# tomisetsu/mochi-db

Hardware: AMD Instinct MI355X
Metric: verified grant signatures/sec (1/2/4/8 GPU) + % of INT32 VALU roofline (higher is better)
Workload: dtype u32

## Files before the change

mochi-db_amd/csrc/capi.cpp:

```cpp
#include <hip/hip_runtime.h>
#include <openssl/bn.h>
#include <openssl/core_names.h>
#include <openssl/evp.h>
#include <openssl/pem.h>

#include <cstdarg>
#include <cstdio>
#include <cstring>
#include <condition_variable>
#include <mutex>
#include <thread>
#include <string>
#include <vector>

#include "../../include/mochi_hip.h"
#include "kernels.h"
#include "mont.h"
#include "w2.h"
#include "w2_encode.h"
#include "w2_host.h"

namespace {

thread_local std::string g_err;
// ... 199 lines not shown
  BN_CTX_free(ctx);
  if (!ok) return fail(MOCHI_EINVAL, "fold matrix precompute failed");
  for (int mt = 0; mt < kFoldMT; mt++)
    for (int ks = 0; ks < kFoldKS; ks++)
      for (int lane = 0; lane < 64; lane++)
        for (int jj = 0; jj < 16; jj++) {
          const int row = 32 * mt + (lane & 31), limb = 8 * ks + 4 * (lane >> 5) + jj / 4;
          if (row < kRows && limb < kFoldNH)
            f->img[((mt * kFoldKS + ks) * 64 + lane) * 16 + jj] = W[(size_t)row * kK + 4 * limb + jj % 4];
        }
  return MOCHI_OK;
}

}

namespace mochi {
const uint32_t* ctx_last_accept_dev(mochi_ctx* c, uint32_t* words, int* device, hipStream_t* stream);
int set_error(int code, const std::string& msg) {
  g_err = msg;
  return code;
}
}

struct mochi_ctx {
  std::mutex ref_mu;
  int batcher_refs = 0;
  bool destroy_pending = false;
  int device = 0;
  hipStream_t stream = nullptr;
  uint32_t n_keys = 0;
  mochi::KeyEntry* d_keys = nullptr;
  mochi::FoldKey* d_fold = nullptr;
  std::mutex mu;
  DevBuf digest, ts, hash_off, hash_len, flags, count, cursor, total, perm, xbuf, dedup, lead;
  DevBuf dev_in, dev_out;
  PinnedBuf pin_in, pin_out;
  hipStream_t s_in = nullptr, s_out = nullptr;
  hipStream_t aux = nullptr;
  hipEvent_t ev_fork = nullptr, ev_join = nullptr;
  hipEvent_t ev_scratch = nullptr;
  bool scratch_used = false;
  hipStream_t scratch_st = nullptr;
  std::vector<hipEvent_t> chunk_ev;
  std::vector<hipEvent_t> tot_ev;
  hipEvent_t evs[2][4] = {{nullptr, nullptr, nullptr, nullptr}, {nullptr, nullptr, nullptr, nullptr}};
  hipEvent_t* ev = evs[0];
  int ev_set = 0, ev_done = 0;
  float last_ms[3] = {0, 0, 0};
  float last_total_ms = 0;
  bool timing_pending = false;
  uint32_t chunk_grants = 0;
  uint32_t small_grants = 4096;
  DevBuf ids, id_off;
  uint32_t n_ids = 0;
  std::vector<std::string> server_ids;
  DevBuf w2_cnt, w2_status, w2_scan, w2_goff, w2_glen, w2_sig, w2_signer, w2_gkey, w2_okey, w2_oflags, w2_sigsrc,
      w2_mgo, w2_ots, w2_okoff, w2_oklen, w2_same;
  PinnedBuf w2_tot;
  hipEvent_t ev_tot = nullptr;
  DevBuf w2e_scratch, w2e_scan;
  PinnedBuf w2e_tot;
  std::vector<hipEvent_t> w2e_ev;
  bool w2e_ev_valid = false;
  const uint32_t* acc_dev = nullptr;
  uint32_t acc_words = 0;
  uint64_t gen = 0;
  bool profiling = false;
// ... 254 lines not shown
  a.blob = b->grant_bytes;
  a.grant_off = b->grant_off;
  a.grant_len = b->grant_len;
  a.sig = b->sig;
  a.signer = b->signer;
  a.grant_key = b->grant_key;
  a.cert_grant_off = b->cert_grant_off;
  a.cert_op_off = b->cert_op_off;
  a.op_key = b->op_key;
  a.op_flags = b->op_flags;
  a.expected_hash = b->expected_hash;
  a.cert_mg_off = b->cert_mg_off;
  a.mg_grant_off = b->mg_grant_off;
  a.op_object_ts = b->op_object_ts;
  a.op_key_off = b->op_key_off;
  a.op_key_len = b->op_key_len;
  a.quorum_mode = p->quorum_mode;
  const uint32_t R = p->replication_factor;
  a.majority = 2 * (R / 3) + 1;
  a.strict_gt = p->strict_gt ? 1 : 0;
  a.keys = c->d_keys;
  a.fold = c->d_fold;
  a.digest = c->digest.as<uint32_t>();
  a.n_dist = N + C;
  a.lead = c->lead.as<uint32_t>();
  a.ts = o->grant_ts ? o->grant_ts : c->ts.as<int64_t>();
  a.hash_off = c->hash_off.as<uint64_t>();
  a.hash_len = c->hash_len.as<uint32_t>();
  a.flags = o->grant_flags ? o->grant_flags : c->flags.as<uint8_t>();
  a.count = c->count.as<uint32_t>();
  a.cursor = c->cursor.as<uint32_t>();
  a.total = c->total.as<uint32_t>();
  a.perm = c->perm.as<uint32_t>();
  a.xbuf = c->xbuf.as<uint32_t>();
  a.rare = c->dedup.as<uint8_t>();
  a.small_grants = c->small_grants;
  a.grant_same = grant_same;
  a.grant_valid_bits = o->grant_valid_bits;
  a.cert_accept_bits = o->cert_accept_bits;
  a.cert_reason = o->cert_reason;
  a.cert_fail_op = o->cert_fail_op;
  a.op_decision = o->op_decision;
  a.op_g0 = o->op_g0;
  a.op_ts = o->op_ts;
  a.op_out_off = op_out_off;
  a.msg_status = msg_status;
  a.aux = prep_serial() ? nullptr : c->aux;
  a.ev_fork = c->ev_fork;
  a.ev_join = c->ev_join;
  if (c->profiling) {
    std::vector<hipEvent_t> evs(2 * mochi::kProfStages, nullptr);
    for (auto& e : evs) HIP_TRY(hipEventCreate(&e));
    c->prof_sets.push_back(evs);
    a.prof_events = c->prof_sets.back().data();
  }
  HIP_TRY(scratch_acquire(c, st));
  HIP_TRY(mochi::launch_verify(a, st));
  HIP_TRY(scratch_release(c, st));
  return MOCHI_OK;
}

bool is_pinned(const void* ptr) {
  if (!ptr) return false;
  hipPointerAttribute_t a;
  if (hipPointerGetAttributes(&a, ptr) != hipSuccess) {
    (void)hipGetLastError();
// ... 2 lines not shown
  return a.type == hipMemoryTypeHost;
}

void par_memcpy(void* dst, const void* src, size_t n) {
  constexpr size_t kPar = 8u << 20;
  if (n < kPar) {
    memcpy(dst, src, n);
    return;
  }
  const unsigned hw = std::thread::hardware_concurrency();
  const unsigned nt = hw < 2 ? 1 : hw > 8 ? 8 : hw;
  const size_t per = (n + nt - 1) / nt;
  std::vector<std::thread> th;
  for (unsigned t = 1; t < nt; t++) {
    const size_t lo = t * per;
    if (lo >= n) break;
    const size_t len = per < n - lo ? per : n - lo;
    th.emplace_back([=] { memcpy((char*)dst + lo, (const char*)src + lo, len); });
  }
  memcpy(dst, src, per < n ? per : n);
  for (auto& x : th) x.join();
}

int ensure_scratch(mochi_ctx* c, uint32_t N, uint32_t C) {
  const uint64_t slots = mochi::slot_capacity(N, c->n_keys);
  const size_t ND = (size_t)N + C;
  int rc;
  if ((rc = c->digest.ensure(sizeof(uint32_t) * 8 * ND)) || (rc = c->dedup.ensure((size_t)N)) ||
      (rc = c->ts.ensure(sizeof(int64_t) * (size_t)N)) || (rc = c->hash_off.ensure(sizeof(uint64_t) * ND)) ||
      (rc = c->hash_len.ensure(sizeof(uint32_t) * ND)) || (rc = c->flags.ensure((size_t)N)) ||
      (rc = c->lead.ensure(sizeof(uint32_t) * (size_t)N)) ||
      (rc = c->count.ensure(sizeof(uint32_t) * c->n_keys)) || (rc = c->cursor.ensure(sizeof(uint32_t) * c->n_keys)) ||
      (rc = c->total.ensure(mochi::kTotalWords * sizeof(uint32_t))) || (rc = c->perm.ensure(sizeof(uint32_t) * (size_t)slots)) ||
      (rc = c->xbuf.ensure(sizeof(uint32_t) * mochi::kL * (size_t)slots)))
    return rc;
  return MOCHI_OK;
}

enum Seg {
  kBlob, kGrantOff, kGrantLen, kSig, kSigner, kGrantKey, kCertGrantOff, kCertOpOff, kOpKey, kOpFlags, kExpHash,
  kCertMgOff, kMgGrantOff, kOpObjTs, kOpKeyOff, kOpKeyLen, kNumSeg
};

int run_host_pipeline(mochi_ctx* c, const mochi_batch* b, const mochi_params* p, mochi_verdicts* o) {
  const uint32_t N = b->n_grants, C = b->n_certs, O = b->n_ops;
  c->acc_dev = nullptr;
  c->acc_words = 0;
  const bool mg = b->cert_mg_off != nullptr;
  struct Chunk {
    uint32_t c0, c1, g0, g1, o0, o1, m0, m1;
    uint64_t lo, hi;
    size_t seg[kNumSeg];
  };
  std::vector<Chunk> ch;
  uint32_t max_grants = 0, max_certs = 0;
  for (uint32_t c0 = 0; c0 < C || (C == 0 && ch.empty());) {
    uint32_t c1 = c0;
    do c1 = c1 + 32 < C ? c1 + 32 : C;
    while (c1 < C && b->cert_grant_off[c1] - b->cert_grant_off[c0] < c->chunk_grants);
    Chunk k{};
    k.c0 = c0;
    k.c1 = c1;
    k.g0 = b->cert_grant_off[c0];
    k.g1 = b->cert_grant_off[c1];
    k.o0 = b->cert_op_off[c0];
    k.o1 = b->cert_op_off[c1];
// ... 991 lines not shown
  c->acc_words = 0;
  return rc;
}

int mochi_fold_matrix(const uint8_t* modulus_be, int8_t* img, uint32_t* cadd) {
  if (!modulus_be || !img || !cadd) return fail(MOCHI_EINVAL, "null argument");
  if (!(modulus_be[0] & 0x80) || !(modulus_be[255] & 1)) return fail(MOCHI_EINVAL, "modulus must be odd, 2048 bits");
  std::vector<mochi::FoldKey> f(1);
  int rc = make_fold_key(modulus_be, f.data());
  if (rc) return rc;
  memcpy(img, f[0].img, sizeof f[0].img);
  memcpy(cadd, f[0].cadd, sizeof f[0].cadd);
  return MOCHI_OK;
}

int mochi_rsa_public_op(mochi_ctx* c, uint32_t n, const uint8_t* sig_be, const uint16_t* signer, uint8_t* out_be,
                        uint32_t* out_z) {
  if (!c || (n && (!sig_be || !signer || !out_be))) return fail(MOCHI_EINVAL, "null argument");
  for (uint32_t i = 0; i < n; i++)
    if (signer[i] >= c->n_keys) return fail(MOCHI_EINVAL, "signer[%u] out of range", i);
  if (n == 0) return MOCHI_OK;
  std::lock_guard<std::mutex> lk(c->mu);
  new_call(c);
  int save = 0;
  (void)hipGetDevice(&save);
  if (hipSetDevice(c->device) != hipSuccess) return fail(MOCHI_EHIP, "hipSetDevice(%d)", c->device);
  const uint64_t slots = mochi::slot_capacity(n, c->n_keys);
  const size_t sig_bytes = (size_t)MOCHI_RSA_BYTES * n, y_bytes = sizeof(uint32_t) * 64 * (size_t)n;
  int rc;
  if ((rc = c->dev_in.ensure(align_up(sig_bytes, 256) + sizeof(uint16_t) * n)) || (rc = c->dev_out.ensure(y_bytes)) ||
      (rc = c->digest.ensure(sizeof(uint32_t) * 8 * (size_t)n)) || (rc = c->flags.ensure(n)) ||
      (rc = c->count.ensure(sizeof(uint32_t) * c->n_keys)) || (rc = c->cursor.ensure(sizeof(uint32_t) * c->n_keys)) ||
      (rc = c->total.ensure(mochi::kTotalWords * sizeof(uint32_t))) || (rc = c->perm.ensure(sizeof(uint32_t) * (size_t)slots)) ||
      (rc = c->xbuf.ensure(sizeof(uint32_t) * mochi::kL * (size_t)slots))) {
    (void)hipSetDevice(save);
    return rc;
  }
  hipStream_t st = c->stream;
  uint8_t* din = c->dev_in.as<uint8_t>();
  uint16_t* dsigner = (uint16_t*)(din + align_up(sig_bytes, 256));
  mochi::LaunchArgs a;
  memset(&a, 0, sizeof a);
  a.n_grants = n;
  a.n_keys = c->n_keys;
  a.n_slots = (uint32_t)slots;
  a.sig = din;
  a.signer = dsigner;
  a.keys = c->d_keys;
  a.fold = c->d_fold;
  a.digest = c->digest.as<uint32_t>();
  a.flags = c->flags.as<uint8_t>();
  a.count = c->count.as<uint32_t>();
  a.cursor = c->cursor.as<uint32_t>();
  a.total = c->total.as<uint32_t>();
  a.perm = c->perm.as<uint32_t>();
  a.xbuf = c->xbuf.as<uint32_t>();
  a.dbg_y = c->dev_out.as<uint32_t>();
  a.skip_prep_tally = true;
  a.small_grants = c->small_grants;
  std::vector<uint32_t> y(64 * (size_t)n), perm, z;
  bool ok = hipMemcpyAsync(din, sig_be, sig_bytes, hipMemcpyHostToDevice, st) == hipSuccess &&
            hipMemcpyAsync(dsigner, signer, sizeof(uint16_t) * n, hipMemcpyHostToDevice, st) == hipSuccess &&
            hipMemsetAsync(a.digest, 0, sizeof(uint32_t) * 8 * (size_t)n, st) == hipSuccess &&
            hipMemsetAsync(a.flags, 0, n, st) == hipSuccess && mochi::launch_verify(a, st) == hipSuccess &&
            hipMemcpyAsync(y.data(), a.dbg_y, y_bytes, hipMemcpyDeviceToHost, st) == hipSuccess;
  if (ok && out_z) {
    perm.resize(slots);
    z.resize((size_t)mochi::kL * slots);
    ok = hipMemcpyAsync(perm.data(), a.perm, sizeof(uint32_t) * slots, hipMemcpyDeviceToHost, st) == hipSuccess &&
         hipMemcpyAsync(z.data(), a.xbuf, sizeof(uint32_t) * z.size(), hipMemcpyDeviceToHost, st) == hipSuccess;
  }
  ok = ok && hipStreamSynchronize(st) == hipSuccess;
  (void)hipSetDevice(save);
  if (!ok) return fail(MOCHI_EHIP, "rsa_public_op failed: %s", hipGetErrorString(hipGetLastError()));
  for (uint32_t g = 0; g < n; g++)
    for (int i = 0; i < 64; i++) {
      const uint32_t w = y[(size_t)g * 64 + i];
      uint8_t* o = out_be + (size_t)g * 256 + 256 - 4 * (i + 1);
      o[0] = (uint8_t)(w >> 24);
      o[1] = (uint8_t)(w >> 16);
      o[2] = (uint8_t)(w >> 8);
      o[3] = (uint8_t)w;
    }
  if (out_z)
    for (uint64_t sl = 0; sl < slots; sl++) {
      const uint32_t g = perm[sl];
      if (g == 0xFFFFFFFFu) continue;
      for (int j = 0; j < mochi::kL; j++) out_z[(size_t)g * mochi::kL + j] = z[(size_t)j * slots + sl];
// ... 404 lines not shown
```

mochi-db_amd/csrc/fold_dev.h:

```cpp
#pragma once
#include <atomic>

#include "fold.h"
#include "kara_dev.h"
#include "mont.h"

namespace mochi {

typedef int v4i __attribute__((ext_vector_type(4)));
typedef int v16i __attribute__((ext_vector_type(16)));

__device__ __forceinline__ void swap32(int& a, int& b) {
  const auto r = __builtin_amdgcn_permlane32_swap(a, b, false, false);
  a = r[0];
  b = r[1];
}

__device__ __forceinline__ int64_t mad_i64(int32_t a, int32_t b, int64_t c) {
  int64_t d;
  uint64_t cc;
  asm("v_mad_i64_i32 %0, %1, %2, %3, %4" : "=v"(d), "=s"(cc) : "v"(a), "s"(b), "v"(c));
  return d;
}

constexpr int kHL = 10;

typedef __attribute__((address_space(1))) char gchar;
typedef __attribute__((address_space(1))) uint32_t guint;

template <bool SUB_H, bool BIASED = false>
__device__ __forceinline__ void fold_reduce(const uint32_t (&t)[2 * kL], uint32_t (&x)[kL],
                                            const v4i* __restrict__ wl, cptr cadd, const uint32_t* hl) {
  v4i a = wl[0];
  v4i b0[kFoldKS], b1[kFoldKS];
// ... 187 lines not shown
        __syncthreads();
        const v4i* src = (const v4i*)fold[key].img;
        for (uint32_t i = threadIdx.x; i < kFoldImgBytes / 16; i += blockDim.x) w[i] = src[i];
        __syncthreads();
        cur_key = key;
      }
      fn(base, key, g_lead);
    }
    if (dyn) {
      it ^= 1;
      if (threadIdx.x == 0) s_grp[it] = nxt;
      __syncthreads();
      grp = __builtin_amdgcn_readfirstlane(s_grp[it]);
    } else {
      grp++;
    }
  }
}

inline uint32_t fold_grid(uint32_t n_slots) {
  static std::atomic<int> n_cu[64];
  int dev = 0;
  (void)hipGetDevice(&dev);
  uint32_t cus = 256u;
  if (dev >= 0 && dev < 64) {
    int v = n_cu[dev].load(std::memory_order_relaxed);
    if (v == 0) {
      if (hipDeviceGetAttribute(&v, hipDeviceAttributeMultiprocessorCount, dev) != hipSuccess || v <= 0) v = 256;
      n_cu[dev].store(v, std::memory_order_relaxed);
    }
    cus = (uint32_t)v;
  }
  const uint32_t groups = (n_slots + kBucketAlign - 1) / kBucketAlign;
  return groups < cus ? groups : cus;
}

}
```

mochi-db_amd/csrc/kernels.h:

```cpp
#pragma once
#include <hip/hip_runtime.h>
#include <stdint.h>

#include "fold.h"

namespace mochi {

struct KeyEntry;

struct LaunchArgs {
  uint32_t n_grants, n_certs, n_keys, n_slots;
  const uint8_t* blob;
  const uint64_t* grant_off;
  const uint32_t* grant_len;
  const uint8_t* sig;
  const uint16_t* signer;
  const uint8_t* grant_key;
  const uint32_t* cert_grant_off;
  const uint32_t* cert_op_off;
  const uint8_t* op_key;
  const uint8_t* op_flags;
  const uint8_t* expected_hash;
  const uint32_t* cert_mg_off;
  const uint32_t* mg_grant_off;
  const int64_t* op_object_ts;
  const uint64_t* op_key_off;
  const uint32_t* op_key_len;
  uint32_t majority, strict_gt, quorum_mode;
  const KeyEntry* keys;
  const FoldKey* fold;
  uint32_t* digest;
  int64_t* ts;
  uint64_t* hash_off;
  uint32_t* hash_len;
  uint32_t* lead;
  uint32_t n_dist;
  uint8_t* flags;
  uint32_t* count;
  uint32_t* cursor;
  uint32_t* total;
  uint8_t* rare;
  const uint32_t* grant_same;
  uint32_t* perm;
  uint32_t* xbuf;
  uint32_t* grant_valid_bits;
  uint32_t* cert_accept_bits;
  uint8_t* cert_reason;
  uint8_t* cert_fail_op;
  uint8_t* op_decision;
  uint32_t* op_g0;
  int64_t* op_ts;
  const uint32_t* op_out_off;
  const uint8_t* msg_status;
  uint32_t* dbg_y;
  bool skip_prep_tally;
  uint32_t small_grants;
  hipStream_t aux;
  hipEvent_t ev_fork, ev_join;
  hipEvent_t* prof_events;
};

enum TotalWord { kTotSlots = 0, kTotPowGroup, kTotFinalGroup, kTotalWords = 4 };

enum ProfStage { kStagePrep = 0, kStageBucket, kStagePow, kStageFinal, kStageTally, kProfStages };

inline uint64_t slot_capacity(uint32_t n_grants, uint32_t n_keys) {
  return (uint64_t)n_grants + (uint64_t)kBucketAlign * (n_keys < n_grants ? n_keys : n_grants);
}

hipError_t launch_verify(const LaunchArgs& a, hipStream_t stream);

size_t sign_key_bytes();
void sign_key_set(void* dst, const uint32_t* p, const uint32_t* q, const uint32_t* r3p, const uint32_t* r3q,
                  const uint32_t* qinv_r, const uint32_t* dp, const uint32_t* dq, const uint32_t* cpad, uint32_t p0inv,
                  uint32_t q0inv, uint32_t dp_bits, uint32_t dq_bits);
hipError_t launch_rsa_sign(const uint8_t* blob, const uint64_t* goff, const uint32_t* glen, uint32_t n,
                           const void* key, uint8_t* sig, uint32_t fault_idx, hipStream_t stream);
hipError_t launch_withhold(const uint8_t* flags, uint32_t n, uint8_t* sig, uint32_t* rejected, hipStream_t stream);
hipError_t launch_pack_bits(const uint8_t* flags, uint32_t n, uint8_t mask, uint32_t* bits, hipStream_t stream);
void launch_rsa_pow(const LaunchArgs& a, hipStream_t stream, bool latency = false);
void launch_rsa_final(const LaunchArgs& a, const uint32_t* lead, uint32_t n_dist, hipStream_t stream,
                      bool latency = false);
void launch_rsa_raw(const LaunchArgs& a, hipStream_t stream);

}
```

mochi-db_amd/csrc/kernels.hip:

```cpp
#include <hip/hip_runtime.h>
#include <stdint.h>
#include <stdlib.h>

#include "../../include/mochi_hip.h"
#include "kernels.h"
#include "prep_dev.h"
#include "proto_dev.h"

namespace mochi {


#ifndef MOCHI_PREP_WAVES
#define MOCHI_PREP_WAVES 4
#endif
#if MOCHI_PREP_WAVES
#define MOCHI_PREP_ATTR __attribute__((amdgpu_waves_per_eu(MOCHI_PREP_WAVES)))
#else
#define MOCHI_PREP_ATTR
#endif
__global__ __launch_bounds__(256) MOCHI_PREP_ATTR void k_grant_prep(const PrepArgs a) {
  const uint32_t i = blockIdx.x * blockDim.x + threadIdx.x;
  if (i < a.n) grant_prep_one(a, i);
}

struct PrepCertArgs {
  const uint8_t* grant_key;
  const uint32_t* cert_grant_off;
  const uint32_t* same;
  uint32_t n_certs;
  uint8_t* rare;
  const uint8_t* expected;
};

__device__ __forceinline__ uint32_t leader_hash_word(const PrepArgs& a, const PrepCertArgs& p, uint32_t c,
                                                     uint64_t og, const PrepOut& o) {
// ... 302 lines not shown
    run += (count[k] + kBucketAlign - 1) & ~(kBucketAlign - 1);
  }
}

#ifndef MOCHI_SCATTER_PER
#define MOCHI_SCATTER_PER 16
#endif
constexpr uint32_t kScatterPer = MOCHI_SCATTER_PER;

__global__ __launch_bounds__(256) void k_bucket_scatter(const uint16_t* __restrict__ signer, uint32_t n, uint32_t n_keys,
                                                        uint32_t* __restrict__ cursor, uint32_t* __restrict__ perm) {
  extern __shared__ uint32_t lds[];
  uint32_t* lcount = lds;
  uint32_t* lbase = lds + n_keys;
  for (uint32_t k = threadIdx.x; k < n_keys; k += blockDim.x) lcount[k] = 0;
  __syncthreads();
  const uint32_t i0 = blockIdx.x * (blockDim.x * kScatterPer) + threadIdx.x;
  uint32_t s[kScatterPer], rank[kScatterPer];
#pragma unroll
  for (uint32_t j = 0; j < kScatterPer; j++) {
    const uint32_t i = i0 + j * blockDim.x;
    uint32_t v = i < n ? (uint32_t)signer[i] : 0xFFFFFFFFu;
    s[j] = v < n_keys ? v : 0xFFFFFFFFu;
  }
#pragma unroll
  for (uint32_t j = 0; j < kScatterPer; j++) rank[j] = wave_counted_add(lcount, s[j]);
  __syncthreads();
  for (uint32_t k = threadIdx.x; k < n_keys; k += blockDim.x)
    lbase[k] = lcount[k] ? atomicAdd(&cursor[k], lcount[k]) : 0u;
  __syncthreads();
#pragma unroll
  for (uint32_t j = 0; j < kScatterPer; j++)
    if (s[j] != 0xFFFFFFFFu) perm[lbase[s[j]] + rank[j]] = i0 + j * blockDim.x;
}

constexpr uint32_t kSmallGrants = 4096;

constexpr uint32_t kSmallPrepFused = 1024;

__global__ __launch_bounds__(1024) void k_bucket_small(const uint16_t* __restrict__ signer, uint32_t n, uint32_t n_keys,
                                                       uint32_t n_slots, uint32_t* __restrict__ perm,
                                                       uint32_t* __restrict__ total, const PrepArgs pa,
                                                       uint32_t prep) {
  extern __shared__ uint32_t lds[];
  uint32_t* cnt = lds;
  uint32_t* cur = lds + n_keys;
  __shared__ uint32_t part[1024];
  for (uint32_t k = threadIdx.x; k < n_keys; k += blockDim.x) cnt[k] = 0;
  for (uint32_t i = threadIdx.x; i < n_slots; i += blockDim.x) perm[i] = 0xFFFFFFFFu;
  __syncthreads();
  for (uint32_t i = threadIdx.x; i < n; i += blockDim.x) {
    const uint32_t k = signer[i];
    if (k < n_keys) atomicAdd(&cnt[k], 1u);
  }
  __syncthreads();
  const uint32_t per = (n_keys + blockDim.x - 1) / blockDim.x, b = threadIdx.x * per;
  uint32_t sum = 0;
  for (uint32_t k = b; k < b + per && k < n_keys; k++) sum += (cnt[k] + kBucketAlign - 1) & ~(kBucketAlign - 1);
  const uint32_t lane = threadIdx.x & 63, wid = threadIdx.x >> 6;
  uint32_t incl = sum;
#pragma unroll
  for (int d = 1; d < 64; d <<= 1) {
    const uint32_t y = __shfl_up(incl, d, 64);
    if (lane >= (uint32_t)d) incl += y;
  }
  if (lane == 63) part[wid] = incl;
// ... 399 lines not shown
  if (n) hipLaunchKernelGGL(k_pack_bits, dim3(cdiv(n, 256)), dim3(256), 0, st, flags, n, mask, bits);
  return hipGetLastError();
}

hipError_t launch_verify(const LaunchArgs& a, hipStream_t st) {
  const uint32_t N = a.n_grants, C = a.n_certs;
  auto mark = [&](int stage, bool end, hipStream_t s) {
    if (a.prof_events) (void)hipEventRecord(a.prof_events[2 * stage + (end ? 1 : 0)], s);
  };
  const bool small = N && N <= a.small_grants && N <= kSmallGrants && !small_off();
  const bool dedup = !small && a.rare && a.lead && a.cert_grant_off && C && !dedup_off();
  const uint32_t nd = a.n_dist ? a.n_dist : N;
  const PrepArgs pa{a.blob,     a.grant_off, a.grant_len, N,        nd,      dedup ? C : 0u,
                    a.digest,   a.ts,        a.hash_off,  a.hash_len, a.flags, dedup ? a.lead : nullptr};
  const uint32_t* lead = dedup ? a.lead : nullptr;
  const bool prep = N && !a.skip_prep_tally;
  const bool fork = prep && a.aux && !small;
  const bool prep_fused = small && prep && N <= kSmallPrepFused && !small_scan_off();
  hipStream_t ps = fork ? a.aux : st;
  auto bucket = [&](hipStream_t bs) -> hipError_t {
    mark(kStageBucket, false, bs);
    if (small) {
      hipLaunchKernelGGL(k_bucket_small, dim3(1), dim3(1024), 2 * sizeof(uint32_t) * a.n_keys, bs, a.signer, N,
                         a.n_keys, a.n_slots, a.perm, a.total, pa, (uint32_t)prep_fused);
    } else if (N) {
      hipError_t e = hipMemsetAsync(a.count, 0, sizeof(uint32_t) * a.n_keys, bs);
      if (e != hipSuccess) return e;
      e = hipMemsetAsync(a.perm, 0xFF, sizeof(uint32_t) * (size_t)a.n_slots, bs);
      if (e != hipSuccess) return e;
      const uint32_t lds = sizeof(uint32_t) * a.n_keys;
      const uint32_t cblocks = cdiv(N, 256) < 1024 ? cdiv(N, 256) : 1024;
      hipLaunchKernelGGL(k_bucket_count, dim3(cblocks), dim3(256), lds, bs, a.signer, N, a.n_keys, a.count);
      hipLaunchKernelGGL(k_bucket_scan, dim3(1), dim3(256), 0, bs, a.count, a.n_keys, a.cursor, a.total);
      hipLaunchKernelGGL(k_bucket_scatter, dim3(cdiv(N, 256 * kScatterPer)), dim3(256), 2 * lds, bs, a.signer, N,
                         a.n_keys, a.cursor, a.perm);
    }
    mark(kStageBucket, true, bs);
    return hipSuccess;
  };
  auto grant_prep = [&](hipStream_t ps) -> hipError_t {
    mark(kStagePrep, false, ps);
    if (prep) {
      if (dedup) {
        const PrepCertArgs pc{a.grant_key, a.cert_grant_off, a.grant_same, C, a.rare,
                              hash_precheck() ? a.expected_hash : nullptr};
        hipError_t e = hipMemsetAsync(a.rare, 1, N, ps);
        if (e != hipSuccess) return e;
        hipLaunchKernelGGL(k_grant_prep_cert, dim3(cdiv(C, 256)), dim3(256), 0, ps, pa, pc);
        const uint32_t mblocks = cdiv(N, 4 * 256) < 2048 ? cdiv(N, 4 * 256) : 2048;
        hipLaunchKernelGGL(k_grant_match, dim3(mblocks), dim3(256), 0, ps, pa, a.rare);
        hipLaunchKernelGGL(k_grant_prep_rare, dim3(cdiv(N, kRareSpan)), dim3(256), 0, ps, pa, (const uint8_t*)a.rare);
      } else if (!prep_fused) {
        hipLaunchKernelGGL(k_grant_prep, dim3(cdiv(N, 256)), dim3(256), 0, ps, pa);
      }
    }
    mark(kStagePrep, true, ps);
    return hipSuccess;
  };
  if (fork && prep_first()) {
    hipError_t e = hipEventRecord(a.ev_fork, st);
    if (e == hipSuccess) e = hipStreamWaitEvent(a.aux, a.ev_fork, 0);
    if (e == hipSuccess) e = bucket(a.aux);
    if (e == hipSuccess) e = hipEventRecord(a.ev_join, a.aux);
    if (e == hipSuccess) e = grant_prep(st);
    if (e == hipSuccess) e = hipStreamWaitEvent(st, a.ev_join, 0);
    if (e != hipSuccess) return e;
// ... 44 lines not shown
    t.op_object_ts = a.op_object_ts;
    t.op_key_off = a.op_key_off;
    t.op_key_len = a.op_key_len;
    t.flags = a.flags;
    t.ts = a.ts;
    t.blob = a.blob;
    t.grant_off = a.grant_off;
    t.grant_len = a.grant_len;
    t.hash_off = a.hash_off;
    t.hash_len = a.hash_len;
    t.lead = lead;
    t.expected = a.expected_hash;
    t.n_certs = C;
    t.majority = a.majority;
    t.strict_gt = a.strict_gt;
    t.quorum_mode = a.quorum_mode;
    t.accept_bits = a.cert_accept_bits;
    t.reason_out = a.cert_reason;
    t.fail_op_out = a.cert_fail_op;
    t.op_decision = a.op_decision;
    t.op_g0 = a.op_g0;
    t.op_ts = a.op_ts;
    t.op_out_off = a.op_out_off;
    t.msg_status = a.msg_status;
    if (dedup && hash_precheck() && !(a.quorum_mode & MOCHI_Q_BIND))
      hipLaunchKernelGGL(k_tally<true>, dim3(cdiv(C, 256)), dim3(256), 0, st, t);
    else
      hipLaunchKernelGGL(k_tally<false>, dim3(cdiv(C, 256)), dim3(256), 0, st, t);
  }
  mark(kStageTally, true, st);
  return hipGetLastError();
}

}
```

mochi-db_amd/csrc/rsa_pow.hip:

```cpp
#include "fold_dev.h"
#include "rsa_common.h"

#include <cstdlib>

#ifndef MOCHI_POW_STAMPS
#define MOCHI_POW_STAMPS 0
#endif
#ifndef MOCHI_POW_DYN
#define MOCHI_POW_DYN 1
#endif
#ifndef MOCHI_LAT_RAW
#define MOCHI_LAT_RAW 0
#endif
#ifndef MOCHI_LAT_ONE_TILE
#define MOCHI_LAT_ONE_TILE 1
#endif
#ifndef MOCHI_POW_NEXT_AHEAD
#define MOCHI_POW_NEXT_AHEAD 1
#endif
#ifndef MOCHI_LAT_STAMPS
#define MOCHI_LAT_STAMPS 0
#endif
namespace mochi {
#if MOCHI_POW_STAMPS
// ... 14 lines not shown
  const uint64_t t = __builtin_amdgcn_s_memtime();
  __builtin_amdgcn_sched_barrier(0);
  return t;
#else
  return 0;
#endif
}

__device__ __forceinline__ uint64_t lstamp() {
#if MOCHI_LAT_STAMPS
  __builtin_amdgcn_sched_barrier(0);
  const uint64_t t = __builtin_amdgcn_s_memtime();
  __builtin_amdgcn_sched_barrier(0);
  return t;
#else
  return 0;
#endif
}

__device__ __forceinline__ void phase_barrier() {
  __builtin_amdgcn_sched_barrier(0);
  __builtin_amdgcn_s_barrier();
  __builtin_amdgcn_sched_barrier(0);
}

struct PowArgs {
  const uint32_t* perm;
  uint32_t n_slots;
  const uint8_t* sig;
  const uint16_t* signer;
  const FoldKey* fold;
  uint32_t* zout;
  uint32_t* ctr;
};

__global__ __launch_bounds__(512, 1) void k_rsa_pow(const PowArgs a) {
  __shared__ v4i w[kFoldImgBytes / 16];
  Stamps st;
  const uint64_t t_begin = stamp();

  const bool lag = __builtin_amdgcn_readfirstlane(threadIdx.x >> 6) >= 4;
  const uint32_t n_groups = (a.n_slots + kBucketAlign - 1) / kBucketAlign;
  uint32_t cur_key = 0xFFFFFFFFu;
#if MOCHI_POW_DYN
  __shared__ uint32_t s_grp[2];
  const bool one_each = n_groups <= gridDim.x;
  if (threadIdx.x == 0) s_grp[0] = one_each ? blockIdx.x : atomicAdd(a.ctr, 1u);
  __syncthreads();
  for (uint32_t it_g = 0;; it_g ^= 1) {
    const uint32_t grp = __builtin_amdgcn_readfirstlane(s_grp[it_g]);
    if (grp >= n_groups) break;
    uint32_t nxt = 0;
    if (threadIdx.x == 0) nxt = one_each ? n_groups : atomicAdd(a.ctr, 1u);
#if !MOCHI_POW_NEXT_AHEAD
    if (threadIdx.x == 0) s_grp[it_g ^ 1] = nxt;
    __syncthreads();
#endif
    auto publish = [&]() {
      if (MOCHI_POW_NEXT_AHEAD && threadIdx.x == 0) s_grp[it_g ^ 1] = nxt;
      __syncthreads();
    };
#else
  const uint32_t g_begin = (uint32_t)((uint64_t)blockIdx.x * n_groups / gridDim.x);
  const uint32_t g_end = (uint32_t)((uint64_t)(blockIdx.x + 1) * n_groups / gridDim.x);
  for (uint32_t grp = g_begin; grp < g_end; grp++) {
#endif
    const uint32_t base = grp * kBucketAlign;
    const uint32_t g_lead = __builtin_amdgcn_readfirstlane(a.perm[base]);
// ... 48 lines not shown
      __builtin_amdgcn_s_setprio(1);
      const uint64_t t2 = stamp();
      fold_reduce<false, true>(t, x, w + (threadIdx.x & 63), ci, nullptr);
      const uint64_t t3 = stamp();
      __builtin_amdgcn_s_setprio(0);
      phase_barrier();
      st.x2 += t1 - t0;
      st.fold += t3 - t2;
      st.n++;
    }
    if (active) {
#pragma unroll
      for (int q = 0; q < kL; q++) a.zout[(size_t)q * a.n_slots + slot] = x[q];
    }
    if (!lag) phase_barrier();
#if MOCHI_POW_DYN
    publish();
#endif
  }
#if MOCHI_POW_STAMPS
  const uint64_t t_end = stamp();
  const uint32_t wv = blockIdx.x * 8 + (threadIdx.x >> 6);
  if ((threadIdx.x & 63) == 0 && wv < 4096) {
    g_pow_stamps[wv][0] = st.x2;
    g_pow_stamps[wv][1] = st.fold;
    g_pow_stamps[wv][2] = t_end - t_begin;
    g_pow_stamps[wv][3] = st.n;
    g_pow_stamps[wv][4] = 0;
  }
#else
  (void)t_begin;
#endif
}

template <int AO, int NOUT, int NA>
__device__ __forceinline__ void lat_square(const uint32_t (&a)[NA], uint32_t (&out)[NOUT]) {
  uint32_t d[kKH];
#pragma unroll
  for (int i = 0; i < kKH; i++) d[i] = a[AO + i] << 1;
  uint64_t col[2 * kKH - 1];
  static_for<0, 2 * kKH - 1>([&](auto kc) {
    constexpr int k = decltype(kc)::value;
    constexpr int lo = k - kKH + 1 > 0 ? k - kKH + 1 : 0;
    constexpr int xhi = k > 0 ? (k - 1) / 2 : -1;
    uint64_t acc = 0;
    if constexpr ((k & 1) == 0) acc = (uint64_t)a[AO + (k >> 1)] * a[AO + (k >> 1)];
    static_for<lo, xhi + 1>([&](auto ic) {
      constexpr int i = decltype(ic)::value;
      acc = mad64(d[i], a[AO + k - i], acc);
    });
    col[k] = acc;
  });
  uint64_t carry = 0;
  static_for<0, NOUT>([&](auto kc) {
    constexpr int k = decltype(kc)::value;
    if constexpr (k < 2 * kKH - 1) {
      const uint64_t v = col[k] + carry;
      out[k] = (uint32_t)v & kLimbMask;
      carry = v >> kLimbBits;
    } else if constexpr (k == 2 * kKH - 1) {
      out[k] = (uint32_t)carry & kLimbMask;
    } else {
      out[k] = (uint32_t)(carry >> kLimbBits);
    }
  });
}
// ... 145 lines not shown
#pragma unroll
    for (int q = 0; q < kL; q++) a.zout[(size_t)q * a.n_slots + slot] = x[q];
  }
}

}

#if MOCHI_POW_STAMPS
extern "C" int mochi_debug_pow_stamps(unsigned long long* out, unsigned n_waves) {
  if (n_waves > 4096) n_waves = 4096;
  return hipMemcpyFromSymbol(out, HIP_SYMBOL(g_pow_stamps), 40 * (size_t)n_waves, 0, hipMemcpyDeviceToHost) == hipSuccess ? 0 : -1;
}
#endif

#if MOCHI_LAT_STAMPS
extern "C" int mochi_debug_lat_stamps(unsigned long long* out, unsigned n_blocks) {
  if (n_blocks > 256) n_blocks = 256;
  return hipMemcpyFromSymbol(out, HIP_SYMBOL(mochi::g_lat_stamps), 256 * (size_t)n_blocks, 0, hipMemcpyDeviceToHost) ==
                 hipSuccess
             ? 0
             : -1;
}
#endif

static bool lat_off() {
  static const bool off = [] {
    const char* e = getenv("MOCHI_NO_LAT");
    return e && e[0] == '1';
  }();
  return off;
}

void launch_rsa_pow(const LaunchArgs& a, hipStream_t st, bool latency) {
  const PowArgs pw{a.perm, a.n_slots, a.sig, a.signer, a.fold, a.xbuf, a.total + kTotPowGroup};
  if (latency && !lat_off()) {
    const uint32_t chunks = (a.n_slots + kLatChunk - 1) / kLatChunk;
    if (chunks) hipLaunchKernelGGL(k_rsa_pow_lat, dim3(chunks), dim3(256), 0, st, pw);
    return;
  }
  const uint32_t blocks = fold_grid(a.n_slots);
  if (blocks) hipLaunchKernelGGL(k_rsa_pow, dim3(blocks), dim3(kBucketAlign), 0, st, pw);
}

}
```

Measured before the change: 366.4 million.

## Precompute per-group descriptors and prefetch next group's signatures in RSA pow kernel

Adds a per-bucket-group descriptor (key and occupancy) computed right after the bucket scan, so the pow kernel no longer has to derive the key and occupancy per group. The restructured k_rsa_pow keeps a three-slot ring of group indices, skips empty groups, and runs padding waves through barriers only. Leading waves prefetch the next group's signature limbs during the post-phase when the key matches, overlapping loads with the lagging waves' work. It also adds an env override for the fold grid size. The cost is an extra small kernel, a descriptor buffer, and more control-flow complexity.

```diff
diff --git a/mochi-db_amd/csrc/capi.cpp b/mochi-db_amd/csrc/capi.cpp
--- a/mochi-db_amd/csrc/capi.cpp
+++ b/mochi-db_amd/csrc/capi.cpp
@@ -255,7 +255,7 @@
   mochi::KeyEntry* d_keys = nullptr;
   mochi::FoldKey* d_fold = nullptr;
   std::mutex mu;
-  DevBuf digest, ts, hash_off, hash_len, flags, count, cursor, total, perm, xbuf, dedup, lead;
+  DevBuf digest, ts, hash_off, hash_len, flags, count, cursor, total, perm, grp_desc, xbuf, dedup, lead;
   DevBuf dev_in, dev_out;
   PinnedBuf pin_in, pin_out;
   hipStream_t s_in = nullptr, s_out = nullptr;
@@ -576,6 +576,7 @@
   a.cursor = c->cursor.as<uint32_t>();
   a.total = c->total.as<uint32_t>();
   a.perm = c->perm.as<uint32_t>();
+  a.grp_desc = c->grp_desc.as<uint32_t>();
   a.xbuf = c->xbuf.as<uint32_t>();
   a.rare = c->dedup.as<uint8_t>();
   a.small_grants = c->small_grants;
@@ -644,6 +645,7 @@
       (rc = c->lead.ensure(sizeof(uint32_t) * (size_t)N)) ||
       (rc = c->count.ensure(sizeof(uint32_t) * c->n_keys)) || (rc = c->cursor.ensure(sizeof(uint32_t) * c->n_keys)) ||
       (rc = c->total.ensure(mochi::kTotalWords * sizeof(uint32_t))) || (rc = c->perm.ensure(sizeof(uint32_t) * (size_t)slots)) ||
+      (rc = c->grp_desc.ensure(sizeof(uint32_t) * mochi::group_count(slots))) ||
       (rc = c->xbuf.ensure(sizeof(uint32_t) * mochi::kL * (size_t)slots)))
     return rc;
   return MOCHI_OK;
@@ -1701,6 +1703,7 @@
       (rc = c->digest.ensure(sizeof(uint32_t) * 8 * (size_t)n)) || (rc = c->flags.ensure(n)) ||
       (rc = c->count.ensure(sizeof(uint32_t) * c->n_keys)) || (rc = c->cursor.ensure(sizeof(uint32_t) * c->n_keys)) ||
       (rc = c->total.ensure(mochi::kTotalWords * sizeof(uint32_t))) || (rc = c->perm.ensure(sizeof(uint32_t) * (size_t)slots)) ||
+      (rc = c->grp_desc.ensure(sizeof(uint32_t) * mochi::group_count(slots))) ||
       (rc = c->xbuf.ensure(sizeof(uint32_t) * mochi::kL * (size_t)slots))) {
     (void)hipSetDevice(save);
     return rc;
@@ -1723,6 +1726,7 @@
   a.cursor = c->cursor.as<uint32_t>();
   a.total = c->total.as<uint32_t>();
   a.perm = c->perm.as<uint32_t>();
+  a.grp_desc = c->grp_desc.as<uint32_t>();
   a.xbuf = c->xbuf.as<uint32_t>();
   a.dbg_y = c->dev_out.as<uint32_t>();
   a.skip_prep_tally = true;
diff --git a/mochi-db_amd/csrc/fold_dev.h b/mochi-db_amd/csrc/fold_dev.h
--- a/mochi-db_amd/csrc/fold_dev.h
+++ b/mochi-db_amd/csrc/fold_dev.h
@@ -1,5 +1,6 @@
 #pragma once
 #include <atomic>
+#include <cstdlib>
 
 #include "fold.h"
 #include "kara_dev.h"
@@ -253,7 +254,12 @@
     cus = (uint32_t)v;
   }
   const uint32_t groups = (n_slots + kBucketAlign - 1) / kBucketAlign;
-  return groups < cus ? groups : cus;
-}
-
-}
+  uint32_t blocks = groups < cus ? groups : cus;
+  if (const char* e = getenv("MOCHI_FOLD_BLOCKS")) {
+    const long n = strtol(e, nullptr, 10);
+    if (n > 0 && (uint64_t)n < blocks) blocks = (uint32_t)n;
+  }
+  return blocks;
+}
+
+}
diff --git a/mochi-db_amd/csrc/kernels.h b/mochi-db_amd/csrc/kernels.h
--- a/mochi-db_amd/csrc/kernels.h
+++ b/mochi-db_amd/csrc/kernels.h
@@ -3,6 +3,10 @@
 #include <stdint.h>
 
 #include "fold.h"
+
+#ifndef MOCHI_GROUP_PIPE
+#define MOCHI_GROUP_PIPE 1
+#endif
 
 namespace mochi {
 
@@ -42,6 +46,7 @@
   uint8_t* rare;
   const uint32_t* grant_same;
   uint32_t* perm;
+  uint32_t* grp_desc;
   uint32_t* xbuf;
   uint32_t* grant_valid_bits;
   uint32_t* cert_accept_bits;
@@ -68,7 +73,71 @@
   return (uint64_t)n_grants + (uint64_t)kBucketAlign * (n_keys < n_grants ? n_keys : n_grants);
 }
 
+inline uint32_t group_count(uint64_t n_slots) { return (uint32_t)((n_slots + kBucketAlign - 1) / kBucketAlign); }
+
+constexpr uint32_t kGrpKeyShift = 16;
+__host__ __device__ inline uint32_t group_desc_key(uint32_t d) { return d >> kGrpKeyShift; }
+__host__ __device__ inline uint32_t group_desc_occupied(uint32_t d) { return d & ((1u << kGrpKeyShift) - 1); }
+
+__host__ __device__ inline uint32_t group_desc(const uint32_t* count, const uint32_t* start, uint32_t n_keys,
+                                               uint32_t g) {
+  const uint32_t base = g * kBucketAlign;
+  uint32_t lo = 0, hi = n_keys;
+  while (lo < hi) {
+    const uint32_t mid = lo + (hi - lo) / 2;
+    if (start[mid] <= base) lo = mid + 1;
+    else hi = mid;
+  }
+  if (lo == 0) return 0;
+  const uint32_t k = lo - 1, off = base - start[k], c = count[k];
+  if (off >= c) return 0;
+  const uint32_t occ = c - off < kBucketAlign ? c - off : kBucketAlign;
+  return (k << kGrpKeyShift) | occ;
+}
+
+struct PowGroupPlan {
+  uint32_t key, occupied;
+  bool empty, restage, padding, load;
+  uint32_t pre_barriers, loop_barriers, post_barriers, spin_barriers;
+  uint32_t block_syncs;
+  __host__ __device__ uint32_t barriers() const {
+    return pre_barriers + loop_barriers + post_barriers + spin_barriers + block_syncs;
+  }
+};
+constexpr uint32_t kPowPhases = 33;
+constexpr uint32_t kNoGroup = 0xFFFFFFFFu;
+__host__ __device__ inline bool pow_wave_has_work(uint32_t desc, uint32_t wave) {
+  return group_desc_occupied(desc) > 64 * wave;
+}
+__host__ __device__ inline PowGroupPlan pow_group_plan(uint32_t desc, uint32_t cur_key, uint32_t wave,
+                                                       bool prefetched) {
+  PowGroupPlan p{};
+  p.key = group_desc_key(desc);
+  p.occupied = group_desc_occupied(desc);
+  p.empty = p.occupied == 0;
+  p.block_syncs = 1;
+  if (p.empty) return p;
+  p.restage = p.key != cur_key;
+  if (p.restage) p.block_syncs += 2;
+  p.padding = !pow_wave_has_work(desc, wave);
+  if (p.padding) {
+    p.spin_barriers = kPowPhases;
+    return p;
+  }
+  const bool lag = wave >= 4;
+  p.pre_barriers = lag ? 1 : 0;
+  p.loop_barriers = kPowPhases - 1;
+  p.post_barriers = lag ? 0 : 1;
+  p.load = !prefetched;
+  return p;
+}
+__host__ __device__ inline bool pow_prefetch_next(uint32_t desc, uint32_t next_desc, uint32_t wave) {
+  return wave < 4 && next_desc != kNoGroup && group_desc_occupied(next_desc) != 0 &&
+         group_desc_key(next_desc) == group_desc_key(desc) && pow_wave_has_work(next_desc, wave);
+}
+
 hipError_t launch_verify(const LaunchArgs& a, hipStream_t stream);
+void launch_group_desc_perm(const LaunchArgs& a, hipStream_t stream);
 
 size_t sign_key_bytes();
 void sign_key_set(void* dst, const uint32_t* p, const uint32_t* q, const uint32_t* r3p, const uint32_t* r3q,
diff --git a/mochi-db_amd/csrc/kernels.hip b/mochi-db_amd/csrc/kernels.hip
--- a/mochi-db_amd/csrc/kernels.hip
+++ b/mochi-db_amd/csrc/kernels.hip
@@ -1,6 +1,8 @@
 #include <hip/hip_runtime.h>
 #include <stdint.h>
 #include <stdlib.h>
+
+#include <vector>
 
 #include "../../include/mochi_hip.h"
 #include "kernels.h"
@@ -369,6 +371,27 @@
 #pragma unroll
   for (uint32_t j = 0; j < kScatterPer; j++)
     if (s[j] != 0xFFFFFFFFu) perm[lbase[s[j]] + rank[j]] = i0 + j * blockDim.x;
+}
+
+__global__ __launch_bounds__(256) void k_bucket_desc(const uint32_t* __restrict__ count,
+                                                     const uint32_t* __restrict__ start, uint32_t n_keys,
+                                                     uint32_t n_groups, uint32_t* __restrict__ grp_desc) {
+  const uint32_t g = blockIdx.x * blockDim.x + threadIdx.x;
+  if (g < n_groups) grp_desc[g] = group_desc(count, start, n_keys, g);
+}
+
+__global__ __launch_bounds__(256) void k_group_desc_perm(const uint32_t* __restrict__ perm, uint32_t n_slots,
+                                                         const uint16_t* __restrict__ signer, uint32_t n_groups,
+                                                         uint32_t* __restrict__ grp_desc) {
+  const uint32_t g = blockIdx.x * (blockDim.x >> 6) + (threadIdx.x >> 6), lane = threadIdx.x & 63;
+  if (g >= n_groups) return;
+  const uint32_t base = g * kBucketAlign;
+  uint32_t occ = 0;
+  for (uint32_t j = 0; j < kBucketAlign; j += 64) {
+    const uint32_t slot = base + j + lane;
+    occ += (uint32_t)__popcll(__ballot(slot < n_slots && perm[slot] != 0xFFFFFFFFu));
+  }
+  if (lane == 0) grp_desc[g] = occ ? ((uint32_t)signer[perm[base]] << kGrpKeyShift) | occ : 0u;
 }
 
 constexpr uint32_t kSmallGrants = 4096;
@@ -834,6 +857,11 @@
       const uint32_t cblocks = cdiv(N, 256) < 1024 ? cdiv(N, 256) : 1024;
       hipLaunchKernelGGL(k_bucket_count, dim3(cblocks), dim3(256), lds, bs, a.signer, N, a.n_keys, a.count);
       hipLaunchKernelGGL(k_bucket_scan, dim3(1), dim3(256), 0, bs, a.count, a.n_keys, a.cursor, a.total);
+#if MOCHI_GROUP_PIPE
+      const uint32_t n_groups = group_count(a.n_slots);
+      hipLaunchKernelGGL(k_bucket_desc, dim3(cdiv(n_groups, 256)), dim3(256), 0, bs, a.count, a.cursor, a.n_keys,
+                         n_groups, a.grp_desc);
+#endif
       hipLaunchKernelGGL(k_bucket_scatter, dim3(cdiv(N, 256 * kScatterPer)), dim3(256), 2 * lds, bs, a.signer, N,
                          a.n_keys, a.cursor, a.perm);
     }
@@ -944,4 +972,34 @@
   return hipGetLastError();
 }
 
-}
+void launch_group_desc_perm(const LaunchArgs& a, hipStream_t st) {
+  const uint32_t n_groups = group_count(a.n_slots);
+  if (n_groups)
+    hipLaunchKernelGGL(k_group_desc_perm, dim3(cdiv(n_groups, 4)), dim3(256), 0, st, a.perm, a.n_slots, a.signer,
+                       n_groups, a.grp_desc);
+}
+
+}
+
+extern "C" int mochi_debug_group_desc(const uint32_t* count, uint32_t n_keys, uint32_t n_groups, uint32_t* out) {
+  if ((n_keys && !count) || (n_groups && !out)) return -1;
+  std::vector<uint32_t> start(n_keys);
+  uint32_t run = 0;
+  for (uint32_t k = 0; k < n_keys; k++) {
+    start[k] = run;
+    run += (count[k] + mochi::kBucketAlign - 1) & ~(mochi::kBucketAlign - 1);
+  }
+  for (uint32_t g = 0; g < n_groups; g++) out[g] = mochi::group_desc(count, start.data(), n_keys, g);
+  return 0;
+}
+
+extern "C" int mochi_debug_pow_plan(uint32_t desc, uint32_t cur_key, uint32_t wave, uint32_t next_desc,
+                                    int prefetched, uint32_t* out) {
+  if (!out || wave >= 8) return -1;
+  const mochi::PowGroupPlan p = mochi::pow_group_plan(desc, cur_key, wave, prefetched != 0);
+  const bool pf = !p.empty && !p.padding && mochi::pow_prefetch_next(desc, next_desc, wave);
+  const uint32_t v[12] = {p.key, p.occupied,     p.empty,         p.restage,       p.padding,       p.load,
+                          pf,    p.pre_barriers, p.loop_barriers, p.post_barriers, p.spin_barriers, p.block_syncs};
+  for (int i = 0; i < 12; i++) out[i] = v[i];
+  return 0;
+}
diff --git a/mochi-db_amd/csrc/rsa_pow.hip b/mochi-db_amd/csrc/rsa_pow.hip
--- a/mochi-db_amd/csrc/rsa_pow.hip
+++ b/mochi-db_amd/csrc/rsa_pow.hip
@@ -70,8 +70,153 @@
   const FoldKey* fold;
   uint32_t* zout;
   uint32_t* ctr;
+  const uint32_t* grp_desc;
 };
 
+#if MOCHI_GROUP_PIPE
+#if !MOCHI_POW_NEXT_AHEAD
+#error "MOCHI_GROUP_PIPE takes group indices ahead: build -DMOCHI_POW_NEXT_AHEAD=0 with -DMOCHI_GROUP_PIPE=0"
+#endif
+static_assert(kPowPhases == 2 * 16 + 1, "16 squarings of two phases, one phase of skew");
+
+__device__ __forceinline__ void pow_load_x(const PowArgs& a, uint32_t base, uint32_t occ, uint32_t (&x)[kL]) {
+  uint32_t g = 0;
+  if (threadIdx.x < occ) g = a.perm[base + threadIdx.x];
+  const uint32_t g0 = __builtin_amdgcn_readfirstlane(g);
+  uint32_t wd[64];
+  load_sig_words(a.sig, threadIdx.x < occ ? g : g0, wd);
+  words_to_limbs(wd, x);
+}
+
+__device__ __forceinline__ void pow_forget_x(uint32_t (&x)[kL]) {
+#pragma unroll
+  for (int q = 0; q < kL; q++) asm volatile("" : "=v"(x[q]));
+}
+
+__global__ __launch_bounds__(512, 1) void k_rsa_pow(const PowArgs a) {
+  __shared__ v4i w[kFoldImgBytes / 16];
+  Stamps st;
+  const uint64_t t_begin = stamp();
+  const uint32_t wave = __builtin_amdgcn_readfirstlane(threadIdx.x >> 6);
+  const uint32_t n_groups = (a.n_slots + kBucketAlign - 1) / kBucketAlign;
+  const cptr desc = as_const(a.grp_desc);
+  uint32_t cur_key = 0xFFFFFFFFu;
+  bool pre = false;
+  uint32_t x[kL];
+#if MOCHI_POW_DYN
+  __shared__ uint32_t s_grp[3];
+  const bool one_each = n_groups <= gridDim.x;
+  auto take = [&]() -> uint32_t { return one_each ? n_groups : atomicAdd(a.ctr, 1u); };
+  if (threadIdx.x == 0) {
+    const uint32_t g0 = one_each ? blockIdx.x : atomicAdd(a.ctr, 1u), g1 = take();
+    s_grp[0] = g0;
+    s_grp[1] = g1;
+  }
+  __syncthreads();
+  uint32_t r0 = 0, r1 = 1, r2 = 2;
+  auto rotate = [&]() {
+    const uint32_t t = r0;
+    r0 = r1, r1 = r2, r2 = t;
+  };
+  for (;; rotate()) {
+    const uint32_t grp = __builtin_amdgcn_readfirstlane(s_grp[r0]);
+    if (grp >= n_groups) break;
+    auto next_group = [&]() -> uint32_t { return __builtin_amdgcn_readfirstlane(s_grp[r1]); };
+    auto put_after_next = [&](uint32_t v) { s_grp[r2] = v; };
+#else
+  const uint32_t g_begin = (uint32_t)((uint64_t)blockIdx.x * n_groups / gridDim.x);
+  const uint32_t g_end = (uint32_t)((uint64_t)(blockIdx.x + 1) * n_groups / gridDim.x);
+  auto take = [&]() -> uint32_t { return 0; };
+  for (uint32_t grp = g_begin; grp < g_end; grp++) {
+    auto next_group = [&]() -> uint32_t { return grp + 1 < g_end ? grp + 1 : n_groups; };
+    auto put_after_next = [&](uint32_t) {};
+#endif
+    const uint32_t d = desc[grp];
+    const PowGroupPlan p = pow_group_plan(d, cur_key, wave, pre);
+    if (p.empty) {
+      if (threadIdx.x == 0) put_after_next(take());
+      __syncthreads();
+      pow_forget_x(x);
+      continue;
+    }
+    if (p.restage) {
+      __syncthreads();
+      const v4i* src = (const v4i*)a.fold[p.key].img;
+      for (uint32_t i = threadIdx.x; i < kFoldImgBytes / 16; i += blockDim.x) w[i] = src[i];
+      __syncthreads();
+      cur_key = p.key;
+    }
+    if (p.padding) {
+#pragma unroll 1
+      for (uint32_t i = 0; i < p.spin_barriers; i++) phase_barrier();
+      __syncthreads();
+      pow_forget_x(x);
+      continue;
+    }
+    const uint32_t base = grp * kBucketAlign;
+    if (p.load) pow_load_x(a, base, p.occupied, x);
+    if (p.pre_barriers) phase_barrier();
+    const cptr c = as_const(a.fold[p.key].cadd);
+#pragma unroll 1
+    for (int it = 0; it < 16; it++) {
+      cptr ci = c;
+      asm volatile("" : "+s"(ci));
+      uint32_t t[2 * kL];
+      const uint64_t t0 = stamp();
+#if MOCHI_KARA2 >= 4
+      kara_square2_lockstep(x, t);
+#elif MOCHI_KARA2
+      kara_square2(x, t);
+#else
+      kara_square(x, t);
+#endif
+      const uint64_t t1 = stamp();
+      phase_barrier();
+      __builtin_amdgcn_s_setprio(1);
+      const uint64_t t2 = stamp();
+      fold_reduce<false, true>(t, x, w + (threadIdx.x & 63), ci, nullptr);
+      const uint64_t t3 = stamp();
+      __builtin_amdgcn_s_setprio(0);
+      phase_barrier();
+      st.x2 += t1 - t0;
+      st.fold += t3 - t2;
+      st.n++;
+    }
+    if (threadIdx.x < p.occupied) {
+#pragma unroll
+      for (int q = 0; q < kL; q++) a.zout[(size_t)q * a.n_slots + base + threadIdx.x] = x[q];
+    }
+    pre = false;
+    pow_forget_x(x);
+    if (p.post_barriers) {
+      uint32_t after = 0;
+      if (threadIdx.x == 0) after = take();
+      const uint32_t nx = next_group();
+      const uint32_t nd = nx < n_groups ? desc[nx] : kNoGroup;
+      if (pow_prefetch_next(d, nd, wave)) {
+        pow_load_x(a, nx * kBucketAlign, group_desc_occupied(nd), x);
+        pre = true;
+      }
+      if (threadIdx.x == 0) put_after_next(after);
+      phase_barrier();
+    }
+    __syncthreads();
+  }
+#if MOCHI_POW_STAMPS
+  const uint64_t t_end = stamp();
+  const uint32_t wv = blockIdx.x * 8 + (threadIdx.x >> 6);
+  if ((threadIdx.x & 63) == 0 && wv < 4096) {
+    g_pow_stamps[wv][0] = st.x2;
+    g_pow_stamps[wv][1] = st.fold;
+    g_pow_stamps[wv][2] = t_end - t_begin;
+    g_pow_stamps[wv][3] = st.n;
+    g_pow_stamps[wv][4] = 0;
+  }
+#else
+  (void)t_begin;
+#endif
+}
+#else
 __global__ __launch_bounds__(512, 1) void k_rsa_pow(const PowArgs a) {
   __shared__ v4i w[kFoldImgBytes / 16];
   Stamps st;
@@ -186,6 +331,7 @@
   (void)t_begin;
 #endif
 }
+#endif
 
 template <int AO, int NOUT, int NA>
 __device__ __forceinline__ void lat_square(const uint32_t (&a)[NA], uint32_t (&out)[NOUT]) {
@@ -397,12 +543,15 @@
 }
 
 void launch_rsa_pow(const LaunchArgs& a, hipStream_t st, bool latency) {
-  const PowArgs pw{a.perm, a.n_slots, a.sig, a.signer, a.fold, a.xbuf, a.total + kTotPowGroup};
+  const PowArgs pw{a.perm, a.n_slots, a.sig, a.signer, a.fold, a.xbuf, a.total + kTotPowGroup, a.grp_desc};
   if (latency && !lat_off()) {
     const uint32_t chunks = (a.n_slots + kLatChunk - 1) / kLatChunk;
     if (chunks) hipLaunchKernelGGL(k_rsa_pow_lat, dim3(chunks), dim3(256), 0, st, pw);
     return;
   }
+#if MOCHI_GROUP_PIPE
+  if (latency) launch_group_desc_perm(a, st);
+#endif
   const uint32_t blocks = fold_grid(a.n_slots);
   if (blocks) hipLaunchKernelGGL(k_rsa_pow, dim3(blocks), dim3(kBucketAlign), 0, st, pw);
 }
```

After: 368.0 million, median of 6. Within noise of the previous version (+0.4%).
